# airl-iisc/MRFP

Measured on AMD Instinct MI355X. Metric: train images/sec, higher is better.
Workload: dtype bf16; 1 GPU; resnet-101 DeepLabV3+ + MRFP+ (HRFP+NP+ on, HRFP re-drawn every step), 768x768, 16 images/GPU, fwd+bwd+SGD, synthetic 19-class, random-init weights; global_batch=16, parallelism=dp1

## Files before the change

### mrfp_amd/csrc/conv_igemm.hip

```cpp
#include "conv_common.hpp"
#include <type_traits>

namespace mrfp {

MRFP_STAMP_DECL(g_stamps_igemm)
int stamps_igemm(unsigned long long* out, int n) { return MRFP_STAMP_READ(g_stamps_igemm, out, n); }

template <typename T, int WM, int WN, bool ALIGNED, bool STRIDED, int TM, int TN, bool RR = false, int ACT = 0>
__global__ __launch_bounds__(64 * WM * WN, ((RR && TM * TN >= 6) ? 2 : 3)) void conv_igemm_kernel(ConvP p) {
    constexpr int NT = 64 * WM * WN, BM = 32 * TM * WM, BN = 32 * TN * WN;
    constexpr int SA = BM * 8 / NT, SB = BN * 8 / NT, RSTEP = NT / 8;
    extern __shared__ __attribute__((aligned(16))) char smem[];
    char* const sA0 = smem;
    char* const sB0 = smem + BM * 128;
    MRFP_STAMP_BEGIN();

    const int t = threadIdx.x, lane = t & 63, wave = t >> 6;
    const int wm = wave / WN, wn = wave % WN;
    const int ntn = (p.N + BN - 1) / BN;
    const int tile = xcd_remap(blockIdx.x, gridDim.x);
    const int m0 = (tile / ntn) * BM, n0 = (tile % ntn) * BN;
    const int rbase = t >> 3;
    const int chunk = (t & 7) ^ ((rbase >> 1) & 7);
    const int wrow = __builtin_amdgcn_readfirstlane(wave) * 8;
// ... 385 lines not shown
            if (mlog < p.M && n < p.N) {
                int m = mlog;
                if (classed) {
                    int b, oh, ow;
                    pixel_of(mlog, b, oh, ow);
                    m = (b * p.Ho + oh) * p.Wo + ow;
                }
                uint4 v = *reinterpret_cast<const uint4*>(epr + row * EPITCH + ch * 16);
                const int mquad = m;
#pragma unroll 1
                for (int qd = 0; qd < (quad ? 4 : 1); ++qd) {
                if (qd > 0) {
                    m = mquad + (qd >> 1) * p.Wo + (qd & 1);
                    v = make_uint4(0u, 0u, 0u, 0u);
                }
                T* dst = y + (size_t)m * p.ldy + n;
                const bool full = n + EPC <= p.N;
                if (p.addend) {
                    const T* ad = reinterpret_cast<const T*>(p.addend) + (size_t)m * p.ldy + n;
                    uint4 av = make_uint4(0u, 0u, 0u, 0u);
                    if (full) {
                        av = *reinterpret_cast<const uint4*>(ad);
                    } else {
#pragma unroll
                        for (int u = 0; u < EPC; ++u)
                            if (n + u < p.N) chunk_set<T>(av, u, ad[u]);
                    }
                    if constexpr (sizeof(T) == 2) {
                        if (p.addend_mask) av = gate_chunk16(av, p.addend_mask[((size_t)m * p.ldy + n) >> 3]);
                    }
                    v = chunk_add<T>(v, av);
                }
                if constexpr (ACT != 0) v = chunk_act<T, ACT>(v);
                if (full) {
                    *reinterpret_cast<uint4*>(dst) = v;
                } else {
#pragma unroll
                    for (int u = 0; u < EPC; ++u)
                        if (n + u < p.N) dst[u] = chunk_get<T>(v, u);
                }
                }
            }
        }
        if constexpr (WIDE) __syncthreads();
        else asm volatile("s_waitcnt lgkmcnt(0)" ::: "memory");
    }
    if (p.colstats) {
        float* out = p.colstats + (size_t)((tile / ntn) * WM + wm) * 2 * p.ldy;
        if constexpr (M16) {
#pragma unroll
            for (int j = 0; j < 2 * TN; ++j) {
                float s2 = cs[j] + __shfl_xor(cs[j], 16, 64), q2 = cq[j] + __shfl_xor(cq[j], 16, 64);
                s2 += __shfl_xor(s2, 32, 64);
                q2 += __shfl_xor(q2, 32, 64);
                const int n = nb + j * 16 + l15;
                if (lq == 0 && n < p.N) {
                    out[n] = s2;
                    out[p.ldy + n] = q2;
                }
            }
        } else
#pragma unroll
        for (int j = 0; j < TN; ++j) {
            const float s2 = cs[j] + __shfl_xor(cs[j], 32, 64), q2 = cq[j] + __shfl_xor(cq[j], 32, 64);
            const int n = nb + j * 32 + lr;
            if (lh == 0 && n < p.N) {
                out[n] = s2;
                out[p.ldy + n] = q2;
            }
        }
    }
}

constexpr int kStatGroups = 64;
constexpr int kCompactAbove = 2048;
__global__ __launch_bounds__(256) void compact_stats_kernel(float* __restrict__ st, int nblk, int C2) {
    __shared__ float part[4][64];
    const int tx = threadIdx.x & 63, ty = threadIdx.x >> 6;
    const int c = blockIdx.x * 64 + tx, g = blockIdx.y;
    const int per = (nblk + kStatGroups - 1) / kStatGroups;
    const int r0 = g * per, r1 = min(nblk, r0 + per);
    const int q = (r1 - r0 + 3) / 4;
    const int a = min(r1, r0 + ty * q), b = min(r1, a + q);
    float a0 = 0.f, a1 = 0.f, a2 = 0.f, a3 = 0.f;
    if (c < C2) {
        int r = a;
        for (; r + 3 < b; r += 4) {
            a0 += st[(size_t)r * C2 + c];
            a1 += st[(size_t)(r + 1) * C2 + c];
            a2 += st[(size_t)(r + 2) * C2 + c];
            a3 += st[(size_t)(r + 3) * C2 + c];
        }
        for (; r < b; ++r) a0 += st[(size_t)r * C2 + c];
    }
    part[ty][tx] = (a0 + a1) + (a2 + a3);
    __syncthreads();
    if (ty == 0 && c < C2) st[(size_t)(nblk + g) * C2 + c] = (part[0][tx] + part[1][tx]) + (part[2][tx] + part[3][tx]);
}

template <typename T, int WM, int WN, bool ALIGNED, bool STRIDED, int TM, int TN, int ACT = 0>
static int launch_igemm(const ConvP& p, hipStream_t st) {
    constexpr int BM = 32 * TM * WM, BN = 32 * TN * WN;
    constexpr int EP = WM * WN * 32 * (32 * TN * (int)sizeof(T) + 16);
    const int lds = (BM + BN) * 128 > EP ? (BM + BN) * 128 : EP;
    static bool attr_set = false;
    if (!attr_set) {
        (void)hipFuncSetAttribute(reinterpret_cast<const void*>(&conv_igemm_kernel<T, WM, WN, ALIGNED, STRIDED, TM, TN, false, ACT>),
                                  hipFuncAttributeMaxDynamicSharedMemorySize, lds);
        attr_set = true;
    }
    const int64_t tiles = (int64_t)((p.M + BM - 1) / BM) * ((p.N + BN - 1) / BN);
    hipLaunchKernelGGL((conv_igemm_kernel<T, WM, WN, ALIGNED, STRIDED, TM, TN, false, ACT>), dim3((unsigned)tiles), dim3(64 * WM * WN), lds, st, p);
    MRFP_LAUNCH_CHECK();
    return 0;
}

template <typename T, int WM, int WN, int TM, int TN, int ACT = 0>
static int launch_igemm_rr(const ConvP& p, hipStream_t st) {
    constexpr int BM = 32 * TM * WM, BN = 32 * TN * WN;
    constexpr int EP = WM * WN * 32 * (32 * TN * (int)sizeof(T) + 16);
    const int fill = (BM + 32 + 3 * BN) * 128;
    const int lds = fill > EP ? fill : EP;
    static bool attr_set = false;
    if (!attr_set) {
        (void)hipFuncSetAttribute(reinterpret_cast<const void*>(&conv_igemm_kernel<T, WM, WN, true, false, TM, TN, true, ACT>),
                                  hipFuncAttributeMaxDynamicSharedMemorySize, lds);
        attr_set = true;
    }
    const int64_t tiles = (int64_t)((p.M + BM - 1) / BM) * ((p.N + BN - 1) / BN);
    hipLaunchKernelGGL((conv_igemm_kernel<T, WM, WN, true, false, TM, TN, true, ACT>), dim3((unsigned)tiles),
                       dim3(64 * WM * WN), lds, st, p);
    MRFP_LAUNCH_CHECK();
    return 0;
}

template <typename T, int WM, int WN, int TM, int TN, int ACT = 0>
static int pick_igemm(const ConvP& p, hipStream_t st) {
    const bool aligned = (p.cpr & 7) == 0, strided = p.sstride > 1;
    if constexpr (ACT != 0) {
        return aligned ? launch_igemm<T, WM, WN, true, false, TM, TN, ACT>(p, st) : launch_igemm<T, WM, WN, false, false, TM, TN, ACT>(p, st);
    }
    if (aligned) return strided ? launch_igemm<T, WM, WN, true, true, TM, TN>(p, st) : launch_igemm<T, WM, WN, true, false, TM, TN>(p, st);
    return strided ? launch_igemm<T, WM, WN, false, true, TM, TN>(p, st) : launch_igemm<T, WM, WN, false, false, TM, TN>(p, st);
}

static bool use_tile96(const ConvP& p, int esz) {
    static const int mode = env_switch("MRFP_CONV_T96", 1);
    if (!mode || p.N <= 64) return false;
    if (mode == 2) return true;
    if (p.sstride > 1) return false;
    const int64_t n128 = (p.N + 127) / 128;
    const int64_t t128 = ((p.M + 127) / 128) * n128, t96 = ((p.M + 95) / 96) * n128;
    const int nkt = (p.kchunks + 7) >> 3;
    if (t96 <= 1024) return true;
    if (nkt > 8) return false;
    const int64_t c128 = ((t128 + 767) / 768) * 128, c96 = ((t96 + 1023) / 1024) * 96;
    return c96 * 10 <= c128 * 9;
}
static bool use_tile192(const ConvP& p, int esz) {
    static const int mode = env_switch("MRFP_CONV_T192", 1);
    if (!mode || esz != 2 || p.N <= 64) return false;
    if (mode == 2) return true;
    if (p.sstride > 1) return false;
    {
        const int64_t t192 = ((int64_t)(p.M + 191) / 192) * ((p.N + 127) / 128);
        if (p.sstride == 1 && (p.cpr & 7) == 0 && p.M % 192 == 0 && t192 % 768 == 0 && t192 <= 3072) return true;
    }
    if (use_tile96(p, esz)) return false;
    const int nkt = (p.kchunks + 7) >> 3;
    return nkt >= 9 && ((p.M + 191) / 192) * ((p.N + 127) / 128) >= 2048;
}


static int rr_tile(const ConvP& p, int esz) {
    static const int mode = env_switch("MRFP_CONV_RR", 2);
    if (!mode || esz != 2) return 0;
    if (p.R != 3 || p.S != 3 || p.stride != 1 || p.sstride != 1 || p.Ho != p.H || p.Wo != p.W) return 0;
// ... 257 lines not shown
```

### mrfp_amd/csrc/stats.hip

```cpp
#include "common.hpp"

namespace mrfp {

static thread_local char g_err[512] = "";
void set_error(const char* fmt, ...) {
    va_list ap;
    va_start(ap, fmt);
    vsnprintf(g_err, sizeof(g_err), fmt, ap);
    va_end(ap);
}

template <typename T, int VEC, int MODE, bool RESIZE, bool YM = false>
__global__ __launch_bounds__(kThreads) void stats_kernel(const T* __restrict__ x, const T* __restrict__ dy,
                                                         const T* __restrict__ y, const float* __restrict__ mean,
                                                         const float* __restrict__ fA, const float* __restrict__ fS,
                                                         int per_image, RowGeom g, int ly, float* __restrict__ ws) {
    __shared__ float sm[kThreads * 2 * VEC];
    const int b = blockIdx.x / ly, j = blockIdx.x % ly;
    const Lanes L = make_lanes(g.C, VEC);
    const int t = threadIdx.x;
    const int tcol = t % L.colthreads, trow = t / L.colthreads;
    const bool active = trow < L.rowthreads;
    float* out = ws + (size_t)blockIdx.x * 2 * g.C;

// ... 53 lines not shown
                            }
                        } else {
                            float dv[VEC], yv[VEC];
                            cvt_f<T, VEC>(dr[u], dv);
                            if (use_y) {
                                cvt_f<T, VEC>(yr[u], yv);
                            } else {
#pragma unroll
                                for (int i = 0; i < VEC; ++i) yv[i] = 1.f;
                            }
#pragma unroll
                            for (int i = 0; i < VEC; ++i) {
                                const float gate = YM ? (((mb[u] >> i) & 1u) ? 1.f : 0.f)
                                                      : use_y ? yv[i] : (remask ? xv[i] * fa[i] + fs[i] : 1.f);
                                const float d = (inside && gate > 0.f) ? dv[i] : 0.f;
                                s[i] += d;
                                q[i] += d * (xv[i] - mu[i]);
                            }
                        }
                    }
                }
            }
        }
        __syncthreads();
#pragma unroll
        for (int i = 0; i < VEC; ++i) {
            sm[(t * 2 + 0) * VEC + i] = s[i];
            sm[(t * 2 + 1) * VEC + i] = q[i];
        }
        __syncthreads();
        const int nout = L.colthreads * 2 * VEC;
        for (int o = t; o < nout; o += kThreads) {
            const int oc = o / (2 * VEC), rest = o % (2 * VEC);
            if (cv0 + oc < L.lpr) {
                float acc = 0.f;
                for (int r = 0; r < L.rowthreads; ++r) acc += sm[((r * L.colthreads + oc) * 2) * VEC + rest];
                const int stat = rest / VEC, i = rest % VEC;
                out[(size_t)stat * g.C + (size_t)(cv0 + oc) * VEC + i] = acc;
            }
        }
    }
}

template <typename T, int MODE>
static int launch_stats(const void* x, const void* dy, const void* y, const float* mean, const float* fA,
                        const float* fS, int per_image,
                        int64_t B, int64_t Ho, int64_t Wo, int64_t C, int64_t Hs, int64_t Ws,
                        const int32_t* tabH, const int32_t* tabW, float* ws, hipStream_t st, bool ymask = false) {
    RowGeom g{(int)B, (int)Ho, (int)Wo, (int)C, (int)Hs, (int)Ws, tabH, tabW};
    const int ly = lines_per_image(B, Ho);
    dim3 grid((unsigned)(B * ly));
    const bool vec_ok = pick_vec<T>(C) > 1 && aligned16(x) && (MODE == 0 || (aligned16(dy) && (y == nullptr || ymask || aligned16(y))));
    const bool resize = tabH != nullptr || tabW != nullptr;
    if (resize && !(tabH && tabW)) { set_error("stats: both index tables or none"); return -1; }
    if (ymask) {
        if constexpr (MODE == 1 && FullVec<T>::value == 8) {
            if (!(vec_ok && !resize && y)) { set_error("stats_bwd_mask: 16-bit activations, C %% 8 == 0, identity geometry"); return -1; }
            hipLaunchKernelGGL((stats_kernel<T, 8, 1, false, true>), grid, dim3(kThreads), 0, st, (const T*)x, (const T*)dy, (const T*)y, mean,
                               fA, fS, per_image, g, ly, ws);
            MRFP_LAUNCH_CHECK();
            return 0;
        } else {
            set_error("stats_bwd_mask: 16-bit activations only");
            return -1;
        }
    }
    auto launch = [&](auto rs) {
        constexpr bool RS = decltype(rs)::value != 0;
        MRFP_LAUNCH_VEC(vec_ok, (stats_kernel<T, FullVec<T>::value, MODE, RS>), (stats_kernel<T, 1, MODE, RS>), grid, st, (const T*)x,
                        (const T*)dy, (const T*)y, mean, fA, fS, per_image, g, ly, ws);
        return 0;
    };
    return resize ? launch(Int<1>{}) : launch(Int<0>{});
}

struct Red { double s, q; };

#ifndef MRFP_FC
#define MRFP_FC 8
#define MRFP_FL 128
#endif
constexpr int kFC = MRFP_FC, kFL = MRFP_FL;
constexpr int kFold = 8;
__device__ __forceinline__ Red reduce_partials(const float* ws, int64_t first, int64_t n, int64_t C, int c, bool valid,
                                               double (*sm)[2][kFC]) {
    const int ty = threadIdx.y, tx = threadIdx.x;
    double s = 0.0, q = 0.0;
    if (valid) {
        float fs[4] = {0.f, 0.f, 0.f, 0.f}, fq[4] = {0.f, 0.f, 0.f, 0.f};
        int64_t p = first + ty;
        for (; p + 3 * kFL < first + n; p += 4 * kFL) {
#pragma unroll
            for (int u = 0; u < 4; ++u) {
                fs[u] = ws[((p + u * kFL) * 2 + 0) * C + c];
                fq[u] = ws[((p + u * kFL) * 2 + 1) * C + c];
            }
#pragma unroll
            for (int u = 0; u < 4; ++u) { s += (double)fs[u]; q += (double)fq[u]; }
        }
        for (; p < first + n; p += kFL) {
            s += (double)ws[(p * 2 + 0) * C + c];
            q += (double)ws[(p * 2 + 1) * C + c];
        }
    }
    __syncthreads();
    sm[ty][0][tx] = s;
    sm[ty][1][tx] = q;
    __syncthreads();
    double s1 = 0.0, q1 = 0.0;
    if (ty < kFL / kFold) {
#pragma unroll
        for (int k = 0; k < kFold; ++k) { s1 += sm[ty * kFold + k][0][tx]; q1 += sm[ty * kFold + k][1][tx]; }
    }
    __syncthreads();
    if (ty < kFL / kFold) { sm[ty][0][tx] = s1; sm[ty][1][tx] = q1; }
    __syncthreads();
    Red r{0.0, 0.0};
    if (ty == 0) {
#pragma unroll
        for (int k = 0; k < kFL / kFold; ++k) { r.s += sm[k][0][tx]; r.q += sm[k][1][tx]; }
    }
    return r;
}

__global__ void bn_finalize_kernel(const float* ws, int64_t nparts, double count, int C, const float* weight,
                                   const float* bias, float eps, float momentum, float* running_mean,
                                   float* running_var, float* mean, float* invstd, float* A, float* S) {
    __shared__ double sm[kFL][2][kFC];
    const int c = blockIdx.x * kFC + threadIdx.x;
    const bool valid = c < C;
    Red r = reduce_partials(ws, 0, nparts, C, c, valid, sm);
    if (threadIdx.y == 0 && valid) {
        const double m = r.s / count;
        double var = r.q / count - m * m;
        if (var < 0.0) var = 0.0;
        const double is = 1.0 / sqrt(var + (double)eps);
        const float w = weight ? weight[c] : 1.f, bb = bias ? bias[c] : 0.f;
        mean[c] = (float)m;
        invstd[c] = (float)is;
        const float a = (float)(w * is);
        A[c] = a;
        S[c] = (float)(bb - m * (double)a);
        if (running_mean) {
            const double unb = count > 1.0 ? var * count / (count - 1.0) : var;
            running_mean[c] = (float)((1.0 - momentum) * running_mean[c] + momentum * m);
            running_var[c] = (float)((1.0 - momentum) * running_var[c] + momentum * unb);
        }
    }
}

__global__ void bn_eval_coef_kernel(int C, const float* weight, const float* bias, const float* rm, const float* rv,
                                    float eps, float* A, float* S) {
    const int c = blockIdx.x * blockDim.x + threadIdx.x;
    if (c >= C) return;
    const float is = 1.0f / sqrtf(rv[c] + eps);
    const float a = (weight ? weight[c] : 1.f) * is;
    A[c] = a;
    S[c] = (bias ? bias[c] : 0.f) - rm[c] * a;
}

__device__ __forceinline__ void norm_bwd_coef(double Ss, double Sq, double count, float w, float mean, float invstd,
                                              float& P, float& Q, float& R) {
    const double is = invstd;
    const double p = (double)w * is;
    const double qq = -(double)w * is * is * is * Sq / count;
    P = (float)p;
    Q = (float)qq;
    R = (float)(-p * Ss / count - qq * (double)mean);
}

__global__ void bn_bwd_finalize_kernel(const float* ws, int64_t nparts, double count, int C, const float* weight,
                                       const float* mean, const float* invstd, float* dweight, float* dbias,
                                       float* P, float* Q, float* R) {
    __shared__ double sm[kFL][2][kFC];
    const int c = blockIdx.x * kFC + threadIdx.x;
    const bool valid = c < C;
    Red r = reduce_partials(ws, 0, nparts, C, c, valid, sm);
    if (threadIdx.y == 0 && valid) {
        if (dbias) dbias[c] = (float)r.s;
        if (dweight) dweight[c] = (float)(r.q * (double)invstd[c]);
        norm_bwd_coef(r.s, r.q, count, weight ? weight[c] : 1.f, mean[c], invstd[c], P[c], Q[c], R[c]);
    }
}

__global__ void in_finalize_kernel(const float* ws, int64_t nslab, double count, int C, const float* weight,
                                   const float* bias, float eps, float* mean, float* invstd, float* A, float* S) {
    __shared__ double sm[kFL][2][kFC];
    const int c = blockIdx.x * kFC + threadIdx.x, b = blockIdx.y;
    const bool valid = c < C;
    Red r = reduce_partials(ws, (int64_t)b * nslab, nslab, C, c, valid, sm);
    if (threadIdx.y == 0 && valid) {
        const double m = r.s / count;
        double var = r.q / count - m * m;
        if (var < 0.0) var = 0.0;
        const double is = 1.0 / sqrt(var + (double)eps);
        const size_t o = (size_t)b * C + c;
        mean[o] = (float)m;
        invstd[o] = (float)is;
        const float a = (float)((weight ? weight[c] : 1.f) * is);
        A[o] = a;
        S[o] = (float)((bias ? bias[c] : 0.f) - m * (double)a);
    }
}

constexpr int kIL = 8;
__global__ void in_bwd_finalize_kernel(const float* ws, int B, int64_t nslab, double count, int C, const float* weight,
                                       const float* mean, const float* invstd, float* dweight, float* dbias,
                                       float* P, float* Q, float* R) {
    __shared__ double sm[kFL][2][kFC];
    const int tx = threadIdx.x, ty = threadIdx.y;
    const int c = blockIdx.x * kFC + tx;
    const bool valid = c < C;
    constexpr int G = kFL / kIL;
    const int gi = ty / kIL, gl = ty % kIL;
    double dw = 0.0, db = 0.0;
    for (int b0 = 0; b0 < B; b0 += G) {
        const int b = b0 + gi;
        const bool mine = valid && b < B;
        double s = 0.0, q = 0.0;
        if (mine) {
            const float* base = ws + ((size_t)b * nslab * 2) * C + c;
            int64_t p = gl;
            for (; p + 3 * kIL < nslab; p += 4 * kIL) {
                float fs[4], fq[4];
#pragma unroll
                for (int u = 0; u < 4; ++u) {
                    fs[u] = base[((p + u * kIL) * 2 + 0) * C];
                    fq[u] = base[((p + u * kIL) * 2 + 1) * C];
                }
#pragma unroll
                for (int u = 0; u < 4; ++u) { s += (double)fs[u]; q += (double)fq[u]; }
            }
            for (; p < nslab; p += kIL) {
                s += (double)base[(p * 2 + 0) * C];
                q += (double)base[(p * 2 + 1) * C];
            }
        }
        __syncthreads();
        sm[ty][0][tx] = s;
        sm[ty][1][tx] = q;
        __syncthreads();
        if (gl == 0 && mine) {
            double rs = 0.0, rq = 0.0;
#pragma unroll
            for (int k = 0; k < kIL; ++k) { rs += sm[ty + k][0][tx]; rq += sm[ty + k][1][tx]; }
            const size_t o = (size_t)b * C + c;
            norm_bwd_coef(rs, rq, count, weight ? weight[c] : 1.f, mean[o], invstd[o], P[o], Q[o], R[o]);
            sm[ty][0][tx] = rs;
            sm[ty][1][tx] = rq * (double)invstd[o];
        }
        __syncthreads();
        if (ty == 0 && valid) {
            for (int g = 0; g < G && b0 + g < B; ++g) { db += sm[g * kIL][0][tx]; dw += sm[g * kIL][1][tx]; }
        }
    }
    if (ty == 0 && valid) {
        if (dweight) dweight[c] = (float)dw;
        if (dbias) dbias[c] = (float)db;
    }
}

__global__ void plane_sum_kernel(const float* ws, int64_t nslab, double scale, int C, float* out) {
    __shared__ double sm[kFL][2][kFC];
    const int c = blockIdx.x * kFC + threadIdx.x, b = blockIdx.y;
    const bool valid = c < C;
    Red r = reduce_partials(ws, (int64_t)b * nslab, nslab, C, c, valid, sm);
    if (threadIdx.y == 0 && valid) out[(size_t)b * C + c] = (float)(r.s * scale);
}

template <typename T>
__global__ void cast_out_kernel(const float* in, T* out, int64_t n) {
    const int64_t i = (int64_t)blockIdx.x * blockDim.x + threadIdx.x;
    if (i < n) out[i] = from_f<T>(in[i]);
}

__device__ __forceinline__ float block_max(float v, float* sm) {
    const int t = threadIdx.x;
    sm[t] = v;
    __syncthreads();
    for (int s = kThreads / 2; s > 0; s >>= 1) {
        if (t < s) sm[t] = fmaxf(sm[t], sm[t + s]);
        __syncthreads();
    }
    const float r = sm[0];
    __syncthreads();
    return r;
}
__device__ __forceinline__ double block_sum(double v, double* sm) {
    const int t = threadIdx.x;
    sm[t] = v;
    __syncthreads();
    for (int s = kThreads / 2; s > 0; s >>= 1) {
        if (t < s) sm[t] += sm[t + s];
        __syncthreads();
    }
    const double r = sm[0];
    __syncthreads();
    return r;
}

__global__ __launch_bounds__(kThreads) void np_coef_kernel(int B, int C, const float* alpha, const float* beta_noise,
                                                           const float* mu, float* sigma, float* A, float* S) {
    __shared__ float smf[kThreads];
    float lmax = -INFINITY;
    for (int c = threadIdx.x; c < C; c += kThreads) {
        double m = 0.0;
        for (int b = 0; b < B; ++b) m += (double)mu[(size_t)b * C + c];
        m /= B;
        double v = 0.0;
        for (int b = 0; b < B; ++b) { const double d = (double)mu[(size_t)b * C + c] - m; v += d * d; }
        const float sg = (float)sqrt(v / (double)(B - 1));
        sigma[c] = sg;
        lmax = fmaxf(lmax, sg);
        if (sg != sg) lmax = sg;
    }
    const float M = block_max(lmax, smf);
    for (int c = threadIdx.x; c < C; c += kThreads) {
        const float scale = sigma[c] / M * 1.5f;
        for (int b = 0; b < B; ++b) {
            const size_t o = (size_t)b * C + c;
            const float beta = 1.f + beta_noise[o] * scale;
            A[o] = alpha[o];
            S[o] = (beta - alpha[o]) * mu[o];
        }
    }
}

__global__ __launch_bounds__(kThreads) void np_bwd_coef_kernel(int B, int C, double hw, const float* alpha,
                                                               const float* beta_noise, const float* mu,
                                                               const float* sigma, const float* G, float* K) {
    __shared__ float smf[kThreads];
    __shared__ double smd[kThreads];
    float lmax = -INFINITY;
    for (int c = threadIdx.x; c < C; c += kThreads) lmax = fmaxf(lmax, sigma[c]);
    const float M = block_max(lmax, smf);
    int larg = 0x7fffffff;
    for (int c = threadIdx.x; c < C; c += kThreads)
        if (sigma[c] == M && c < larg) larg = c;
    const int cstar = -(int)block_max(-(float)larg, smf);
    double lt = 0.0;
    for (int c = threadIdx.x; c < C; c += kThreads) {
        double ds = 0.0;
        for (int b = 0; b < B; ++b) {
            const size_t o = (size_t)b * C + c;
            ds += (double)mu[o] * (double)G[o] * (double)beta_noise[o];
        }
        lt += ds * (double)sigma[c];
    }
    const double T = block_sum(lt, smd);
    const double Md = (double)M;
    for (int c = threadIdx.x; c < C; c += kThreads) {
        double ds = 0.0, mbar = 0.0;
        for (int b = 0; b < B; ++b) {
            const size_t o = (size_t)b * C + c;
            ds += (double)mu[o] * (double)G[o] * (double)beta_noise[o];
            mbar += (double)mu[o];
        }
        mbar /= B;
        double dsig = 1.5 * ds / Md;
        if (c == cstar) dsig -= 1.5 * T / (Md * Md);
        const double scale = (double)sigma[c] / Md * 1.5;
        for (int b = 0; b < B; ++b) {
            const size_t o = (size_t)b * C + c;
            const double beta = 1.0 + (double)beta_noise[o] * scale;
            double dmu = (beta - (double)alpha[o]) * (double)G[o];
            dmu += dsig * ((double)mu[o] - mbar) / ((double)(B - 1) * (double)sigma[c]);
            K[o] = (float)(dmu / hw);
        }
    }
}

}

using namespace mrfp;

extern "C" {

int mrfp_version(void) { return 100; }
const char* mrfp_last_error(void) { return mrfp::g_err; }

int64_t mrfp_stats_nslab(int64_t B, int64_t Ho) { return lines_per_image(B, Ho); }

int mrfp_stats_fwd(const void* x, int dtype, int64_t B, int64_t Ho, int64_t Wo, int64_t C, int64_t Hs, int64_t Ws,
                   const int32_t* tabH, const int32_t* tabW, float* ws, void* stream) {
    MRFP_CHECK(x && ws && B > 0 && Ho > 0 && Wo > 0 && C > 0, "stats_fwd: bad arguments");
    MRFP_CHECK(C <= 65536 && B * Ho < (1LL << 31), "stats_fwd: shape out of range");
    hipStream_t st = (hipStream_t)stream;
    return by_dtype(dtype, "stats_fwd", [&](auto t) {
        using T = typename decltype(t)::type;
        return launch_stats<T, 0>(x, nullptr, nullptr, nullptr, nullptr, nullptr, 0, B, Ho, Wo, C, Hs, Ws, tabH, tabW, ws, st);
    });
}

int mrfp_stats_bwd(const void* dy, const void* x, const void* y, const float* mean, const float* fA, const float* fS,
                   int per_image, int dtype,
                   int64_t B, int64_t Ho, int64_t Wo, int64_t C, int64_t Hs, int64_t Ws, const int32_t* tabH,
                   const int32_t* tabW, float* ws, void* stream) {
    MRFP_CHECK(dy && x && ws && B > 0 && Ho > 0 && Wo > 0 && C > 0, "stats_bwd: bad arguments");
    hipStream_t st = (hipStream_t)stream;
    return by_dtype(dtype, "stats_bwd", [&](auto t) {
        using T = typename decltype(t)::type;
        return launch_stats<T, 1>(x, dy, y, mean, fA, fS, per_image, B, Ho, Wo, C, Hs, Ws, tabH, tabW, ws, st);
    });
}

int mrfp_stats_bwd_mask(const void* dy, const void* x, const void* mask, const float* mean, int per_image, int dtype, int64_t B,
                        int64_t H, int64_t W, int64_t C, float* ws, void* stream) {
    MRFP_CHECK(dy && x && mask && ws && B > 0 && H > 0 && W > 0 && C > 0 && (C & 7) == 0, "stats_bwd_mask: bad arguments");
    hipStream_t st = (hipStream_t)stream;
    return by_dtype16(dtype, "stats_bwd_mask", [&](auto t) {
        using T = typename decltype(t)::type;
        return launch_stats<T, 1>(x, dy, mask, mean, nullptr, nullptr, per_image, B, H, W, C, H, W, nullptr, nullptr, ws, st, true);
    });
}

int mrfp_bn_finalize(const float* ws, int64_t B, int64_t nslab, int64_t count, int64_t C, const float* weight,
                     const float* bias, float eps, float momentum, float* running_mean, float* running_var,
                     float* mean, float* invstd, float* A, float* S, void* stream) {
    MRFP_CHECK(ws && mean && invstd && A && S && C > 0 && count > 0, "bn_finalize: bad arguments");
    hipLaunchKernelGGL(bn_finalize_kernel, dim3((unsigned)((C + mrfp::kFC - 1) / mrfp::kFC)), dim3(mrfp::kFC, mrfp::kFL), 0, (hipStream_t)stream, ws,
                       B * nslab, (double)count, (int)C, weight, bias, eps, momentum, running_mean, running_var, mean,
                       invstd, A, S);
    MRFP_LAUNCH_CHECK();
    return 0;
}

int mrfp_bn_eval_coef(int64_t C, const float* weight, const float* bias, const float* running_mean,
                      const float* running_var, float eps, float* A, float* S, void* stream) {
    MRFP_CHECK(running_mean && running_var && A && S && C > 0, "bn_eval_coef: bad arguments");
    hipLaunchKernelGGL(bn_eval_coef_kernel, dim3((unsigned)((C + 255) / 256)), dim3(256), 0, (hipStream_t)stream, (int)C,
                       weight, bias, running_mean, running_var, eps, A, S);
    MRFP_LAUNCH_CHECK();
    return 0;
}

int mrfp_bn_bwd_finalize(const float* ws, int64_t B, int64_t nslab, int64_t count, int64_t C, const float* weight,
                         const float* mean, const float* invstd, float* dweight, float* dbias, float* P, float* Q,
                         float* R, void* stream) {
    MRFP_CHECK(ws && mean && invstd && P && Q && R && C > 0 && count > 0, "bn_bwd_finalize: bad arguments");
    hipLaunchKernelGGL(bn_bwd_finalize_kernel, dim3((unsigned)((C + mrfp::kFC - 1) / mrfp::kFC)), dim3(mrfp::kFC, mrfp::kFL), 0, (hipStream_t)stream, ws,
                       B * nslab, (double)count, (int)C, weight, mean, invstd, dweight, dbias, P, Q, R);
    MRFP_LAUNCH_CHECK();
    return 0;
}

int mrfp_in_finalize(const float* ws, int64_t B, int64_t nslab, int64_t count, int64_t C, const float* weight,
                     const float* bias, float eps, float* mean, float* invstd, float* A, float* S, void* stream) {
    MRFP_CHECK(ws && mean && invstd && A && S && C > 0 && count > 0 && B > 0 && B < 65536, "in_finalize: bad arguments");
    hipLaunchKernelGGL(in_finalize_kernel, dim3((unsigned)((C + mrfp::kFC - 1) / mrfp::kFC), (unsigned)B), dim3(mrfp::kFC, mrfp::kFL), 0,
                       (hipStream_t)stream, ws, nslab, (double)count, (int)C, weight, bias, eps, mean, invstd, A, S);
    MRFP_LAUNCH_CHECK();
    return 0;
}

int mrfp_in_bwd_finalize(const float* ws, int64_t B, int64_t nslab, int64_t count, int64_t C, const float* weight,
                         const float* mean, const float* invstd, float* dweight, float* dbias, float* P, float* Q,
                         float* R, void* stream) {
    MRFP_CHECK(ws && mean && invstd && P && Q && R && C > 0 && count > 0, "in_bwd_finalize: bad arguments");
    hipLaunchKernelGGL(in_bwd_finalize_kernel, dim3((unsigned)((C + mrfp::kFC - 1) / mrfp::kFC)), dim3(mrfp::kFC, mrfp::kFL), 0, (hipStream_t)stream, ws,
                       (int)B, nslab, (double)count, (int)C, weight, mean, invstd, dweight, dbias, P, Q, R);
    MRFP_LAUNCH_CHECK();
    return 0;
}

int mrfp_np_finalize(const float* ws, int64_t B, int64_t nslab, int64_t count, int64_t C, const float* alpha,
                     const float* beta_noise, float* mu, float* sigma, float* A, float* S, void* stream) {
    MRFP_CHECK(ws && alpha && beta_noise && mu && sigma && A && S && C > 0 && B > 0 && B < 65536, "np_finalize: bad arguments");
    hipStream_t st = (hipStream_t)stream;
    hipLaunchKernelGGL(plane_sum_kernel, dim3((unsigned)((C + mrfp::kFC - 1) / mrfp::kFC), (unsigned)B), dim3(mrfp::kFC, mrfp::kFL), 0, st, ws, nslab,
                       1.0 / (double)count, (int)C, mu);
    MRFP_LAUNCH_CHECK();
    hipLaunchKernelGGL(np_coef_kernel, dim3(1), dim3(kThreads), 0, st, (int)B, (int)C, alpha, beta_noise, mu, sigma, A, S);
    MRFP_LAUNCH_CHECK();
    return 0;
}

int mrfp_np_bwd_finalize(const float* ws, int64_t B, int64_t nslab, int64_t count, int64_t C, const float* alpha,
                         const float* beta_noise, const float* mu, const float* sigma, float* Gtmp, float* K,
                         void* stream) {
    MRFP_CHECK(ws && alpha && beta_noise && mu && sigma && Gtmp && K && C > 0 && B > 0 && B < 65536, "np_bwd_finalize: bad arguments");
    hipStream_t st = (hipStream_t)stream;
    hipLaunchKernelGGL(plane_sum_kernel, dim3((unsigned)((C + mrfp::kFC - 1) / mrfp::kFC), (unsigned)B), dim3(mrfp::kFC, mrfp::kFL), 0, st, ws, nslab, 1.0,
                       (int)C, Gtmp);
    MRFP_LAUNCH_CHECK();
    hipLaunchKernelGGL(np_bwd_coef_kernel, dim3(1), dim3(kThreads), 0, st, (int)B, (int)C, (double)count, alpha,
                       beta_noise, mu, sigma, Gtmp, K);
    MRFP_LAUNCH_CHECK();
    return 0;
}

int mrfp_mean_finalize(const float* ws, int64_t B, int64_t nslab, int64_t count, int64_t C, float* tmp, void* out,
                       int dtype, void* stream) {
    MRFP_CHECK(ws && out && tmp && C > 0 && B > 0 && B < 65536, "mean_finalize: bad arguments");
    hipStream_t st = (hipStream_t)stream;
    return by_dtype(dtype, "mean_finalize", [&](auto t) {
        using T = typename decltype(t)::type;
        constexpr bool cast = !std::is_same<T, float>::value;
        hipLaunchKernelGGL(plane_sum_kernel, dim3((unsigned)((C + mrfp::kFC - 1) / mrfp::kFC), (unsigned)B), dim3(mrfp::kFC, mrfp::kFL), 0, st, ws,
                           nslab, 1.0 / (double)count, (int)C, cast ? tmp : (float*)out);
        MRFP_LAUNCH_CHECK();
        if constexpr (cast) {
            const int64_t n = B * C;
            hipLaunchKernelGGL((cast_out_kernel<T>), dim3((unsigned)((n + 255) / 256)), dim3(256), 0, st, tmp, (T*)out, n);
            MRFP_LAUNCH_CHECK();
        }
        return 0;
    });
}

}
```

Baseline: 308.6 images/sec.

## Batch and predicate loads in stat-finalize reductions; use wave-level folds

Rewrites the per-channel partial-stat reduction kernels so each lane issues a fixed batch of clamped, predicated loads, with the batch depth chosen by row count through a templated dispatch. Within-wave folds now use a wave barrier instead of block barriers. Parameter loads are hoisted ahead of the reduction, and the NP coefficient kernels cache per-batch columns in registers. Block reductions switch to shuffle-based wave reductions. The goal is more memory-level parallelism and fewer syncs in small latency-bound finalize kernels, at the cost of more template instances and redundant clamped loads.

```diff
diff --git a/mrfp_amd/csrc/conv_igemm.hip b/mrfp_amd/csrc/conv_igemm.hip
--- a/mrfp_amd/csrc/conv_igemm.hip
+++ b/mrfp_amd/csrc/conv_igemm.hip
@@ -491,17 +491,22 @@
     const int r0 = g * per, r1 = min(nblk, r0 + per);
     const int q = (r1 - r0 + 3) / 4;
     const int a = min(r1, r0 + ty * q), b = min(r1, a + q);
-    float a0 = 0.f, a1 = 0.f, a2 = 0.f, a3 = 0.f;
-    if (c < C2) {
-        int r = a;
-        for (; r + 3 < b; r += 4) {
-            a0 += st[(size_t)r * C2 + c];
-            a1 += st[(size_t)(r + 1) * C2 + c];
-            a2 += st[(size_t)(r + 2) * C2 + c];
-            a3 += st[(size_t)(r + 3) * C2 + c];
-        }
-        for (; r < b; ++r) a0 += st[(size_t)r * C2 + c];
-    }
+    constexpr int kCB = 16;
+    const float* col = st + min(c, C2 - 1);
+    const int full = a + ((b - a) & ~3);
+    float acc[4] = {0.f, 0.f, 0.f, 0.f};
+    for (int r0 = a; r0 < b; r0 += kCB) {
+        float v[kCB];
+#pragma unroll
+        for (int u = 0; u < kCB; ++u) v[u] = col[(size_t)min(r0 + u, nblk - 1) * C2];
+#pragma unroll
+        for (int u = 0; u < kCB; ++u) {
+            const int r = r0 + u;
+            acc[u & 3] = r < full ? acc[u & 3] + v[u] : acc[u & 3];
+            acc[0] = (r >= full && r < b) ? acc[0] + v[u] : acc[0];
+        }
+    }
+    const float a0 = acc[0], a1 = acc[1], a2 = acc[2], a3 = acc[3];
     part[ty][tx] = (a0 + a1) + (a2 + a3);
     __syncthreads();
     if (ty == 0 && c < C2) st[(size_t)(nblk + g) * C2 + c] = (part[0][tx] + part[1][tx]) + (part[2][tx] + part[3][tx]);
diff --git a/mrfp_amd/csrc/stats.hip b/mrfp_amd/csrc/stats.hip
--- a/mrfp_amd/csrc/stats.hip
+++ b/mrfp_amd/csrc/stats.hip
@@ -159,60 +159,98 @@
 #endif
 constexpr int kFC = MRFP_FC, kFL = MRFP_FL;
 constexpr int kFold = 8;
-__device__ __forceinline__ Red reduce_partials(const float* ws, int64_t first, int64_t n, int64_t C, int c, bool valid,
-                                               double (*sm)[2][kFC]) {
-    const int ty = threadIdx.y, tx = threadIdx.x;
-    double s = 0.0, q = 0.0;
-    if (valid) {
-        float fs[4] = {0.f, 0.f, 0.f, 0.f}, fq[4] = {0.f, 0.f, 0.f, 0.f};
-        int64_t p = first + ty;
-        for (; p + 3 * kFL < first + n; p += 4 * kFL) {
-#pragma unroll
-            for (int u = 0; u < 4; ++u) {
-                fs[u] = ws[((p + u * kFL) * 2 + 0) * C + c];
-                fq[u] = ws[((p + u * kFL) * 2 + 1) * C + c];
-            }
-#pragma unroll
-            for (int u = 0; u < 4; ++u) { s += (double)fs[u]; q += (double)fq[u]; }
-        }
-        for (; p < first + n; p += kFL) {
-            s += (double)ws[(p * 2 + 0) * C + c];
-            q += (double)ws[(p * 2 + 1) * C + c];
-        }
-    }
-    __syncthreads();
+constexpr int kFW = kFL / kFold;
+constexpr int kWL = 64 / kFC;
+static_assert(kFC * kWL == 64 && kWL % kFold == 0 && kFL % kWL == 0 && kFC * kFL <= 1024,
+              "finalize block: whole waves, and a wave holds whole groups of kFold partial lanes");
+
+template <int R, int STEP>
+__device__ __forceinline__ void add_rows(const float* __restrict__ col, int64_t p, int64_t n, int64_t C, double& s, double& q) {
+    float fs[R], fq[R];
+#pragma unroll
+    for (int u = 0; u < R; ++u) {
+        const int64_t r = min(p + (int64_t)u * STEP, n - 1);
+        fs[u] = col[(r * 2 + 0) * C];
+        fq[u] = col[(r * 2 + 1) * C];
+    }
+#pragma unroll
+    for (int u = 0; u < R; ++u) {
+        const bool in = p + (int64_t)u * STEP < n;
+        s = in ? s + (double)fs[u] : s;
+        q = in ? q + (double)fq[u] : q;
+    }
+}
+
+template <int STEP, int R>
+__device__ __forceinline__ void sum_lane_rows(const float* __restrict__ col, int lane, int64_t n, int64_t C, double& s, double& q) {
+    s = 0.0;
+    q = 0.0;
+    for (int64_t p0 = 0; p0 < n; p0 += R * STEP) add_rows<R, STEP>(col, p0 + lane, n, C, s, q);
+}
+
+__device__ __forceinline__ bool fold_groups(double s, double q, double (*sm)[2][kFC], int tx, int ty) {
     sm[ty][0][tx] = s;
     sm[ty][1][tx] = q;
-    __syncthreads();
+    __builtin_amdgcn_fence(__ATOMIC_RELEASE, "wavefront");
+    __builtin_amdgcn_wave_barrier();
+    __builtin_amdgcn_fence(__ATOMIC_ACQUIRE, "wavefront");
+    if (ty % kFold != 0) return false;
     double s1 = 0.0, q1 = 0.0;
-    if (ty < kFL / kFold) {
-#pragma unroll
-        for (int k = 0; k < kFold; ++k) { s1 += sm[ty * kFold + k][0][tx]; q1 += sm[ty * kFold + k][1][tx]; }
-    }
-    __syncthreads();
-    if (ty < kFL / kFold) { sm[ty][0][tx] = s1; sm[ty][1][tx] = q1; }
+#pragma unroll
+    for (int k = 0; k < kFold; ++k) { s1 += sm[ty + k][0][tx]; q1 += sm[ty + k][1][tx]; }
+    sm[ty][0][tx] = s1;
+    sm[ty][1][tx] = q1;
+    return true;
+}
+
+template <typename F>
+static void finalize_batch(int64_t n, int lanes, F&& f) {
+    if (n <= 1 * lanes) f(Int<1>{});
+    else if (n <= 2 * lanes) f(Int<2>{});
+    else if (n <= 3 * lanes) f(Int<3>{});
+    else if (n <= 4 * lanes) f(Int<4>{});
+    else if (n <= 6 * lanes) f(Int<6>{});
+    else if (n <= 8 * lanes) f(Int<8>{});
+    else if (n <= 12 * lanes) f(Int<12>{});
+    else f(Int<16>{});
+}
+
+__device__ __forceinline__ float load_or(const float* p, int i, const float* safe, float d) {
+    const float v = *(p ? p + i : safe);
+    return p ? v : d;
+}
+
+template <int R>
+__device__ __forceinline__ Red reduce_partials(const float* ws, int64_t first, int64_t n, int64_t C, int c, double (*sm)[2][kFC]) {
+    const int ty = threadIdx.y, tx = threadIdx.x;
+    double s, q;
+    sum_lane_rows<kFL, R>(ws + first * 2 * C + c, ty, n, C, s, q);
+    fold_groups(s, q, sm, tx, ty);
     __syncthreads();
     Red r{0.0, 0.0};
     if (ty == 0) {
 #pragma unroll
-        for (int k = 0; k < kFL / kFold; ++k) { r.s += sm[k][0][tx]; r.q += sm[k][1][tx]; }
+        for (int k = 0; k < kFW; ++k) { r.s += sm[k * kFold][0][tx]; r.q += sm[k * kFold][1][tx]; }
     }
     return r;
 }
 
-__global__ void bn_finalize_kernel(const float* ws, int64_t nparts, double count, int C, const float* weight,
+template <int NR>
+__global__ __launch_bounds__(kFC * kFL) void bn_finalize_kernel(const float* ws, int64_t nparts, double count, int C, const float* weight,
                                    const float* bias, float eps, float momentum, float* running_mean,
                                    float* running_var, float* mean, float* invstd, float* A, float* S) {
     __shared__ double sm[kFL][2][kFC];
     const int c = blockIdx.x * kFC + threadIdx.x;
     const bool valid = c < C;
-    Red r = reduce_partials(ws, 0, nparts, C, c, valid, sm);
+    const int cl = min(c, C - 1);
+    const float w = load_or(weight, cl, ws, 1.f), bb = load_or(bias, cl, ws, 0.f);
+    const float rm = load_or(running_mean, cl, ws, 0.f), rv = load_or(running_mean ? running_var : nullptr, cl, ws, 0.f);
+    Red r = reduce_partials<NR>(ws, 0, nparts, C, cl, sm);
     if (threadIdx.y == 0 && valid) {
         const double m = r.s / count;
         double var = r.q / count - m * m;
         if (var < 0.0) var = 0.0;
         const double is = 1.0 / sqrt(var + (double)eps);
-        const float w = weight ? weight[c] : 1.f, bb = bias ? bias[c] : 0.f;
         mean[c] = (float)m;
         invstd[c] = (float)is;
         const float a = (float)(w * is);
@@ -220,8 +258,8 @@
         S[c] = (float)(bb - m * (double)a);
         if (running_mean) {
             const double unb = count > 1.0 ? var * count / (count - 1.0) : var;
-            running_mean[c] = (float)((1.0 - momentum) * running_mean[c] + momentum * m);
-            running_var[c] = (float)((1.0 - momentum) * running_var[c] + momentum * unb);
+            running_mean[c] = (float)((1.0 - momentum) * rm + momentum * m);
+            running_var[c] = (float)((1.0 - momentum) * rv + momentum * unb);
         }
     }
 }
@@ -246,26 +284,32 @@
     R = (float)(-p * Ss / count - qq * (double)mean);
 }
 
-__global__ void bn_bwd_finalize_kernel(const float* ws, int64_t nparts, double count, int C, const float* weight,
+template <int NR>
+__global__ __launch_bounds__(kFC * kFL) void bn_bwd_finalize_kernel(const float* ws, int64_t nparts, double count, int C, const float* weight,
                                        const float* mean, const float* invstd, float* dweight, float* dbias,
                                        float* P, float* Q, float* R) {
     __shared__ double sm[kFL][2][kFC];
     const int c = blockIdx.x * kFC + threadIdx.x;
     const bool valid = c < C;
-    Red r = reduce_partials(ws, 0, nparts, C, c, valid, sm);
+    const int cl = min(c, C - 1);
+    const float w = load_or(weight, cl, ws, 1.f), mu = mean[cl], is = invstd[cl];
+    Red r = reduce_partials<NR>(ws, 0, nparts, C, cl, sm);
     if (threadIdx.y == 0 && valid) {
         if (dbias) dbias[c] = (float)r.s;
-        if (dweight) dweight[c] = (float)(r.q * (double)invstd[c]);
-        norm_bwd_coef(r.s, r.q, count, weight ? weight[c] : 1.f, mean[c], invstd[c], P[c], Q[c], R[c]);
-    }
-}
-
-__global__ void in_finalize_kernel(const float* ws, int64_t nslab, double count, int C, const float* weight,
+        if (dweight) dweight[c] = (float)(r.q * (double)is);
+        norm_bwd_coef(r.s, r.q, count, w, mu, is, P[c], Q[c], R[c]);
+    }
+}
+
+template <int NR>
+__global__ __launch_bounds__(kFC * kFL) void in_finalize_kernel(const float* ws, int64_t nslab, double count, int C, const float* weight,
                                    const float* bias, float eps, float* mean, float* invstd, float* A, float* S) {
     __shared__ double sm[kFL][2][kFC];
     const int c = blockIdx.x * kFC + threadIdx.x, b = blockIdx.y;
     const bool valid = c < C;
-    Red r = reduce_partials(ws, (int64_t)b * nslab, nslab, C, c, valid, sm);
+    const int cl = min(c, C - 1);
+    const float w = load_or(weight, cl, ws, 1.f), bb = load_or(bias, cl, ws, 0.f);
+    Red r = reduce_partials<NR>(ws, (int64_t)b * nslab, nslab, C, cl, sm);
     if (threadIdx.y == 0 && valid) {
         const double m = r.s / count;
         double var = r.q / count - m * m;
@@ -274,61 +318,42 @@
         const size_t o = (size_t)b * C + c;
         mean[o] = (float)m;
         invstd[o] = (float)is;
-        const float a = (float)((weight ? weight[c] : 1.f) * is);
+        const float a = (float)(w * is);
         A[o] = a;
-        S[o] = (float)((bias ? bias[c] : 0.f) - m * (double)a);
-    }
-}
-
-constexpr int kIL = 8;
-__global__ void in_bwd_finalize_kernel(const float* ws, int B, int64_t nslab, double count, int C, const float* weight,
+        S[o] = (float)(bb - m * (double)a);
+    }
+}
+
+constexpr int kIL = kFold;
+template <int NR>
+__global__ __launch_bounds__(kFC * kFL) void in_bwd_finalize_kernel(const float* ws, int B, int64_t nslab, double count, int C, const float* weight,
                                        const float* mean, const float* invstd, float* dweight, float* dbias,
                                        float* P, float* Q, float* R) {
-    __shared__ double sm[kFL][2][kFC];
+    constexpr int G = kFL / kIL;
+    __shared__ double sm[2][kFL][2][kFC];
     const int tx = threadIdx.x, ty = threadIdx.y;
     const int c = blockIdx.x * kFC + tx;
     const bool valid = c < C;
-    constexpr int G = kFL / kIL;
+    const int cl = min(c, C - 1);
     const int gi = ty / kIL, gl = ty % kIL;
+    const float w = load_or(weight, cl, ws, 1.f);
     double dw = 0.0, db = 0.0;
-    for (int b0 = 0; b0 < B; b0 += G) {
+    for (int b0 = 0, par = 0; b0 < B; b0 += G, par ^= 1) {
         const int b = b0 + gi;
         const bool mine = valid && b < B;
-        double s = 0.0, q = 0.0;
-        if (mine) {
-            const float* base = ws + ((size_t)b * nslab * 2) * C + c;
-            int64_t p = gl;
-            for (; p + 3 * kIL < nslab; p += 4 * kIL) {
-                float fs[4], fq[4];
-#pragma unroll
-                for (int u = 0; u < 4; ++u) {
-                    fs[u] = base[((p + u * kIL) * 2 + 0) * C];
-                    fq[u] = base[((p + u * kIL) * 2 + 1) * C];
-                }
-#pragma unroll
-                for (int u = 0; u < 4; ++u) { s += (double)fs[u]; q += (double)fq[u]; }
-            }
-            for (; p < nslab; p += kIL) {
-                s += (double)base[(p * 2 + 0) * C];
-                q += (double)base[(p * 2 + 1) * C];
-            }
-        }
-        __syncthreads();
-        sm[ty][0][tx] = s;
-        sm[ty][1][tx] = q;
-        __syncthreads();
-        if (gl == 0 && mine) {
-            double rs = 0.0, rq = 0.0;
-#pragma unroll
-            for (int k = 0; k < kIL; ++k) { rs += sm[ty + k][0][tx]; rq += sm[ty + k][1][tx]; }
+        const size_t ol = (size_t)min(b, B - 1) * C + cl;
+        const float mu = mean[ol], is = invstd[ol];
+        double s, q;
+        sum_lane_rows<kIL, NR>(ws + ((size_t)min(b, B - 1) * nslab * 2) * C + cl, gl, nslab, C, s, q);
+        if (fold_groups(s, q, sm[par], tx, ty) && mine) {
             const size_t o = (size_t)b * C + c;
-            norm_bwd_coef(rs, rq, count, weight ? weight[c] : 1.f, mean[o], invstd[o], P[o], Q[o], R[o]);
-            sm[ty][0][tx] = rs;
-            sm[ty][1][tx] = rq * (double)invstd[o];
+            const double rs = sm[par][ty][0][tx], rq = sm[par][ty][1][tx];
+            norm_bwd_coef(rs, rq, count, w, mu, is, P[o], Q[o], R[o]);
+            sm[par][ty][1][tx] = rq * (double)is;
         }
         __syncthreads();
         if (ty == 0 && valid) {
-            for (int g = 0; g < G && b0 + g < B; ++g) { db += sm[g * kIL][0][tx]; dw += sm[g * kIL][1][tx]; }
+            for (int g = 0; g < G && b0 + g < B; ++g) { db += sm[par][g * kIL][0][tx]; dw += sm[par][g * kIL][1][tx]; }
         }
     }
     if (ty == 0 && valid) {
@@ -337,12 +362,20 @@
     }
 }
 
-__global__ void plane_sum_kernel(const float* ws, int64_t nslab, double scale, int C, float* out) {
+template <int NR>
+__global__ __launch_bounds__(kFC * kFL) void plane_sum_kernel(const float* ws, int64_t nslab, double scale, int C, float* out) {
     __shared__ double sm[kFL][2][kFC];
     const int c = blockIdx.x * kFC + threadIdx.x, b = blockIdx.y;
     const bool valid = c < C;
-    Red r = reduce_partials(ws, (int64_t)b * nslab, nslab, C, c, valid, sm);
+    Red r = reduce_partials<NR>(ws, (int64_t)b * nslab, nslab, C, min(c, C - 1), sm);
     if (threadIdx.y == 0 && valid) out[(size_t)b * C + c] = (float)(r.s * scale);
+}
+
+static void launch_plane_sum(const float* ws, int64_t B, int64_t nslab, double scale, int64_t C, float* out, hipStream_t st) {
+    finalize_batch(nslab, kFL, [&](auto r) {
+        hipLaunchKernelGGL(plane_sum_kernel<decltype(r)::value>, dim3((unsigned)((C + kFC - 1) / kFC), (unsigned)B), dim3(kFC, kFL), 0, st, ws,
+                           nslab, scale, (int)C, out);
+    });
 }
 
 template <typename T>
@@ -351,97 +384,111 @@
     if (i < n) out[i] = from_f<T>(in[i]);
 }
 
+static_assert(kThreads == 256, "block_max / block_sum: four waves");
 __device__ __forceinline__ float block_max(float v, float* sm) {
-    const int t = threadIdx.x;
-    sm[t] = v;
+#pragma unroll
+    for (int s = 32; s > 0; s >>= 1) v = fmaxf(v, __shfl_xor(v, s, 64));
+    if ((threadIdx.x & 63) == 0) sm[threadIdx.x >> 6] = v;
     __syncthreads();
-    for (int s = kThreads / 2; s > 0; s >>= 1) {
-        if (t < s) sm[t] = fmaxf(sm[t], sm[t + s]);
-        __syncthreads();
-    }
-    const float r = sm[0];
+    return fmaxf(fmaxf(sm[0], sm[1]), fmaxf(sm[2], sm[3]));
+}
+__device__ __forceinline__ double block_sum(double v, double* sm) {
+    const int l = threadIdx.x & 63;
+    sm[threadIdx.x] = v;
     __syncthreads();
-    return r;
-}
-__device__ __forceinline__ double block_sum(double v, double* sm) {
-    const int t = threadIdx.x;
-    sm[t] = v;
-    __syncthreads();
-    for (int s = kThreads / 2; s > 0; s >>= 1) {
-        if (t < s) sm[t] += sm[t + s];
-        __syncthreads();
-    }
-    const double r = sm[0];
-    __syncthreads();
-    return r;
-}
-
+    double x = (sm[l] + sm[l + 128]) + (sm[l + 64] + sm[l + 192]);
+#pragma unroll
+    for (int s = 32; s > 0; s >>= 1) x += __shfl_down(x, s, 64);
+    return __shfl(x, 0, 64);
+}
+
+template <int NB>
+struct Col {
+    const float* p;
+    int C;
+    float r[NB ? NB : 1];
+    __device__ __forceinline__ Col(const float* base, int B, int C_, int c) : p(base), C(C_) {
+        if constexpr (NB > 0) {
+#pragma unroll
+            for (int b = 0; b < NB; ++b) r[b] = base[(size_t)min(b, B - 1) * C_ + c];
+        }
+    }
+    __device__ __forceinline__ float at(int b, int c) const {
+        if constexpr (NB > 0) return r[b];
+        else return p[(size_t)b * C + c];
+    }
+};
+#define MRFP_FOR_B(b) _Pragma("unroll") for (int b = 0; b < (NB > 0 ? NB : B); ++b) if (b < B)
+constexpr int kNpB = 16;
+
+template <int NB>
 __global__ __launch_bounds__(kThreads) void np_coef_kernel(int B, int C, const float* alpha, const float* beta_noise,
                                                            const float* mu, float* sigma, float* A, float* S) {
-    __shared__ float smf[kThreads];
-    float lmax = -INFINITY;
+    __shared__ float smf[4];
+    const int cl = min((int)threadIdx.x, C - 1);
+    const Col<NB> cmu(mu, B, C, cl), cal(alpha, B, C, cl), cno(beta_noise, B, C, cl);
+    float lmax = -INFINITY, sg = 0.f;
     for (int c = threadIdx.x; c < C; c += kThreads) {
         double m = 0.0;
-        for (int b = 0; b < B; ++b) m += (double)mu[(size_t)b * C + c];
+        MRFP_FOR_B(b) m += (double)cmu.at(b, c);
         m /= B;
         double v = 0.0;
-        for (int b = 0; b < B; ++b) { const double d = (double)mu[(size_t)b * C + c] - m; v += d * d; }
-        const float sg = (float)sqrt(v / (double)(B - 1));
+        MRFP_FOR_B(b) { const double d = (double)cmu.at(b, c) - m; v += d * d; }
+        sg = (float)sqrt(v / (double)(B - 1));
         sigma[c] = sg;
         lmax = fmaxf(lmax, sg);
         if (sg != sg) lmax = sg;
     }
     const float M = block_max(lmax, smf);
     for (int c = threadIdx.x; c < C; c += kThreads) {
-        const float scale = sigma[c] / M * 1.5f;
-        for (int b = 0; b < B; ++b) {
+        const float scale = (NB > 0 ? sg : sigma[c]) / M * 1.5f;
+        MRFP_FOR_B(b) {
             const size_t o = (size_t)b * C + c;
-            const float beta = 1.f + beta_noise[o] * scale;
-            A[o] = alpha[o];
-            S[o] = (beta - alpha[o]) * mu[o];
-        }
-    }
-}
-
+            const float beta = 1.f + cno.at(b, c) * scale;
+            A[o] = cal.at(b, c);
+            S[o] = (beta - cal.at(b, c)) * cmu.at(b, c);
+        }
+    }
+}
+
+template <int NB>
 __global__ __launch_bounds__(kThreads) void np_bwd_coef_kernel(int B, int C, double hw, const float* alpha,
                                                                const float* beta_noise, const float* mu,
                                                                const float* sigma, const float* G, float* K) {
-    __shared__ float smf[kThreads];
+    __shared__ float smf[2][4];
     __shared__ double smd[kThreads];
+    const int cl = min((int)threadIdx.x, C - 1);
+    const Col<NB> cmu(mu, B, C, cl), cal(alpha, B, C, cl), cno(beta_noise, B, C, cl), cg(G, B, C, cl);
     float lmax = -INFINITY;
     for (int c = threadIdx.x; c < C; c += kThreads) lmax = fmaxf(lmax, sigma[c]);
-    const float M = block_max(lmax, smf);
+    const float M = block_max(lmax, smf[0]);
     int larg = 0x7fffffff;
     for (int c = threadIdx.x; c < C; c += kThreads)
         if (sigma[c] == M && c < larg) larg = c;
-    const int cstar = -(int)block_max(-(float)larg, smf);
+    const int cstar = -(int)block_max(-(float)larg, smf[1]);
     double lt = 0.0;
     for (int c = threadIdx.x; c < C; c += kThreads) {
         double ds = 0.0;
-        for (int b = 0; b < B; ++b) {
-            const size_t o = (size_t)b * C + c;
-            ds += (double)mu[o] * (double)G[o] * (double)beta_noise[o];
-        }
+        MRFP_FOR_B(b) ds += (double)cmu.at(b, c) * (double)cg.at(b, c) * (double)cno.at(b, c);
         lt += ds * (double)sigma[c];
     }
     const double T = block_sum(lt, smd);
     const double Md = (double)M;
     for (int c = threadIdx.x; c < C; c += kThreads) {
         double ds = 0.0, mbar = 0.0;
-        for (int b = 0; b < B; ++b) {
-            const size_t o = (size_t)b * C + c;
-            ds += (double)mu[o] * (double)G[o] * (double)beta_noise[o];
-            mbar += (double)mu[o];
+        MRFP_FOR_B(b) {
+            ds += (double)cmu.at(b, c) * (double)cg.at(b, c) * (double)cno.at(b, c);
+            mbar += (double)cmu.at(b, c);
         }
         mbar /= B;
         double dsig = 1.5 * ds / Md;
         if (c == cstar) dsig -= 1.5 * T / (Md * Md);
         const double scale = (double)sigma[c] / Md * 1.5;
-        for (int b = 0; b < B; ++b) {
+        MRFP_FOR_B(b) {
             const size_t o = (size_t)b * C + c;
-            const double beta = 1.0 + (double)beta_noise[o] * scale;
-            double dmu = (beta - (double)alpha[o]) * (double)G[o];
-            dmu += dsig * ((double)mu[o] - mbar) / ((double)(B - 1) * (double)sigma[c]);
+            const double beta = 1.0 + (double)cno.at(b, c) * scale;
+            double dmu = (beta - (double)cal.at(b, c)) * (double)cg.at(b, c);
+            dmu += dsig * ((double)cmu.at(b, c) - mbar) / ((double)(B - 1) * (double)sigma[c]);
             K[o] = (float)(dmu / hw);
         }
     }
@@ -495,9 +542,10 @@
                      const float* bias, float eps, float momentum, float* running_mean, float* running_var,
                      float* mean, float* invstd, float* A, float* S, void* stream) {
     MRFP_CHECK(ws && mean && invstd && A && S && C > 0 && count > 0, "bn_finalize: bad arguments");
-    hipLaunchKernelGGL(bn_finalize_kernel, dim3((unsigned)((C + mrfp::kFC - 1) / mrfp::kFC)), dim3(mrfp::kFC, mrfp::kFL), 0, (hipStream_t)stream, ws,
-                       B * nslab, (double)count, (int)C, weight, bias, eps, momentum, running_mean, running_var, mean,
-                       invstd, A, S);
+    finalize_batch(B * nslab, mrfp::kFL, [&](auto r) {
+        hipLaunchKernelGGL(bn_finalize_kernel<decltype(r)::value>, dim3((unsigned)((C + mrfp::kFC - 1) / mrfp::kFC)), dim3(mrfp::kFC, mrfp::kFL), 0, (hipStream_t)stream, ws, B * nslab, (double)count,
+                           (int)C, weight, bias, eps, momentum, running_mean, running_var, mean, invstd, A, S);
+    });
     MRFP_LAUNCH_CHECK();
     return 0;
 }
@@ -515,8 +563,10 @@
                          const float* mean, const float* invstd, float* dweight, float* dbias, float* P, float* Q,
                          float* R, void* stream) {
     MRFP_CHECK(ws && mean && invstd && P && Q && R && C > 0 && count > 0, "bn_bwd_finalize: bad arguments");
-    hipLaunchKernelGGL(bn_bwd_finalize_kernel, dim3((unsigned)((C + mrfp::kFC - 1) / mrfp::kFC)), dim3(mrfp::kFC, mrfp::kFL), 0, (hipStream_t)stream, ws,
-                       B * nslab, (double)count, (int)C, weight, mean, invstd, dweight, dbias, P, Q, R);
+    finalize_batch(B * nslab, mrfp::kFL, [&](auto r) {
+        hipLaunchKernelGGL(bn_bwd_finalize_kernel<decltype(r)::value>, dim3((unsigned)((C + mrfp::kFC - 1) / mrfp::kFC)), dim3(mrfp::kFC, mrfp::kFL), 0, (hipStream_t)stream, ws, B * nslab,
+                           (double)count, (int)C, weight, mean, invstd, dweight, dbias, P, Q, R);
+    });
     MRFP_LAUNCH_CHECK();
     return 0;
 }
@@ -524,8 +574,10 @@
 int mrfp_in_finalize(const float* ws, int64_t B, int64_t nslab, int64_t count, int64_t C, const float* weight,
                      const float* bias, float eps, float* mean, float* invstd, float* A, float* S, void* stream) {
     MRFP_CHECK(ws && mean && invstd && A && S && C > 0 && count > 0 && B > 0 && B < 65536, "in_finalize: bad arguments");
-    hipLaunchKernelGGL(in_finalize_kernel, dim3((unsigned)((C + mrfp::kFC - 1) / mrfp::kFC), (unsigned)B), dim3(mrfp::kFC, mrfp::kFL), 0,
-                       (hipStream_t)stream, ws, nslab, (double)count, (int)C, weight, bias, eps, mean, invstd, A, S);
+    finalize_batch(nslab, mrfp::kFL, [&](auto r) {
+        hipLaunchKernelGGL(in_finalize_kernel<decltype(r)::value>, dim3((unsigned)((C + mrfp::kFC - 1) / mrfp::kFC), (unsigned)B), dim3(mrfp::kFC, mrfp::kFL), 0, (hipStream_t)stream, ws, nslab, (double)count, (int)C,
+                           weight, bias, eps, mean, invstd, A, S);
+    });
     MRFP_LAUNCH_CHECK();
     return 0;
 }
@@ -534,8 +586,10 @@
                          const float* mean, const float* invstd, float* dweight, float* dbias, float* P, float* Q,
                          float* R, void* stream) {
     MRFP_CHECK(ws && mean && invstd && P && Q && R && C > 0 && count > 0, "in_bwd_finalize: bad arguments");
-    hipLaunchKernelGGL(in_bwd_finalize_kernel, dim3((unsigned)((C + mrfp::kFC - 1) / mrfp::kFC)), dim3(mrfp::kFC, mrfp::kFL), 0, (hipStream_t)stream, ws,
-                       (int)B, nslab, (double)count, (int)C, weight, mean, invstd, dweight, dbias, P, Q, R);
+    finalize_batch(nslab, mrfp::kIL, [&](auto r) {
+        hipLaunchKernelGGL(in_bwd_finalize_kernel<decltype(r)::value>, dim3((unsigned)((C + mrfp::kFC - 1) / mrfp::kFC)), dim3(mrfp::kFC, mrfp::kFL), 0, (hipStream_t)stream, ws, (int)B, nslab,
+                           (double)count, (int)C, weight, mean, invstd, dweight, dbias, P, Q, R);
+    });
     MRFP_LAUNCH_CHECK();
     return 0;
 }
@@ -544,10 +598,12 @@
                      const float* beta_noise, float* mu, float* sigma, float* A, float* S, void* stream) {
     MRFP_CHECK(ws && alpha && beta_noise && mu && sigma && A && S && C > 0 && B > 0 && B < 65536, "np_finalize: bad arguments");
     hipStream_t st = (hipStream_t)stream;
-    hipLaunchKernelGGL(plane_sum_kernel, dim3((unsigned)((C + mrfp::kFC - 1) / mrfp::kFC), (unsigned)B), dim3(mrfp::kFC, mrfp::kFL), 0, st, ws, nslab,
-                       1.0 / (double)count, (int)C, mu);
-    MRFP_LAUNCH_CHECK();
-    hipLaunchKernelGGL(np_coef_kernel, dim3(1), dim3(kThreads), 0, st, (int)B, (int)C, alpha, beta_noise, mu, sigma, A, S);
+    launch_plane_sum(ws, B, nslab, 1.0 / (double)count, C, mu, st);
+    MRFP_LAUNCH_CHECK();
+    if (B <= kNpB && C <= kThreads)
+        hipLaunchKernelGGL(np_coef_kernel<kNpB>, dim3(1), dim3(kThreads), 0, st, (int)B, (int)C, alpha, beta_noise, mu, sigma, A, S);
+    else
+        hipLaunchKernelGGL(np_coef_kernel<0>, dim3(1), dim3(kThreads), 0, st, (int)B, (int)C, alpha, beta_noise, mu, sigma, A, S);
     MRFP_LAUNCH_CHECK();
     return 0;
 }
@@ -557,11 +613,14 @@
                          void* stream) {
     MRFP_CHECK(ws && alpha && beta_noise && mu && sigma && Gtmp && K && C > 0 && B > 0 && B < 65536, "np_bwd_finalize: bad arguments");
     hipStream_t st = (hipStream_t)stream;
-    hipLaunchKernelGGL(plane_sum_kernel, dim3((unsigned)((C + mrfp::kFC - 1) / mrfp::kFC), (unsigned)B), dim3(mrfp::kFC, mrfp::kFL), 0, st, ws, nslab, 1.0,
-                       (int)C, Gtmp);
-    MRFP_LAUNCH_CHECK();
-    hipLaunchKernelGGL(np_bwd_coef_kernel, dim3(1), dim3(kThreads), 0, st, (int)B, (int)C, (double)count, alpha,
-                       beta_noise, mu, sigma, Gtmp, K);
+    launch_plane_sum(ws, B, nslab, 1.0, C, Gtmp, st);
+    MRFP_LAUNCH_CHECK();
+    if (B <= kNpB && C <= kThreads)
+        hipLaunchKernelGGL(np_bwd_coef_kernel<kNpB>, dim3(1), dim3(kThreads), 0, st, (int)B, (int)C, (double)count, alpha,
+                           beta_noise, mu, sigma, Gtmp, K);
+    else
+        hipLaunchKernelGGL(np_bwd_coef_kernel<0>, dim3(1), dim3(kThreads), 0, st, (int)B, (int)C, (double)count, alpha,
+                           beta_noise, mu, sigma, Gtmp, K);
     MRFP_LAUNCH_CHECK();
     return 0;
 }
@@ -573,8 +632,7 @@
     return by_dtype(dtype, "mean_finalize", [&](auto t) {
         using T = typename decltype(t)::type;
         constexpr bool cast = !std::is_same<T, float>::value;
-        hipLaunchKernelGGL(plane_sum_kernel, dim3((unsigned)((C + mrfp::kFC - 1) / mrfp::kFC), (unsigned)B), dim3(mrfp::kFC, mrfp::kFL), 0, st, ws,
-                           nslab, 1.0 / (double)count, (int)C, cast ? tmp : (float*)out);
+        launch_plane_sum(ws, B, nslab, 1.0 / (double)count, C, cast ? tmp : (float*)out, st);
         MRFP_LAUNCH_CHECK();
         if constexpr (cast) {
             const int64_t n = B * C;
```

Result: no change. 308.5 images/sec (-0.0%).
